# congkaishen/MotionPlanning

Measured on AMD Instinct MI355X. Metric: MPPI rollouts/s (K×H dyn+cost steps/s) at K=8192,H=50; 1/2/4/8 GPU, higher is better.
Workload: dtype f64

## Files before the change

motionplanning_amd/csrc/mppi.hip:

```cpp
#include "mppi_device.hpp"
#include "mppi_plan.hpp"
#include "runtime.hpp"

#include <hip/hip_ext.h>

#include <algorithm>
#include <cstdlib>
#include <type_traits>
#include <vector>

using namespace mpk;

namespace {

constexpr int NT = 256;
constexpr int RPB = NT / 2;

__device__ __forceinline__ double block_reduce_min(double v, double* sh) {
  for (int o = 32; o >= 1; o >>= 1) v = nanmin(v, __shfl_xor(v, o));
  const int w = threadIdx.x >> 6;
  __syncthreads();
  if ((threadIdx.x & 63) == 0) sh[w] = v;
  __syncthreads();
  double r = sh[0];
  for (int i = 1; i < (int)(blockDim.x >> 6); i++) r = nanmin(r, sh[i]);
  __syncthreads();
  return r;
}

__device__ __forceinline__ double block_reduce_sum(double v, double* sh) {
  for (int o = 32; o >= 1; o >>= 1) v = v + __shfl_xor(v, o);
  const int w = threadIdx.x >> 6;
  __syncthreads();
  if ((threadIdx.x & 63) == 0) sh[w] = v;
  __syncthreads();
  double r = sh[0];
  for (int i = 1; i < (int)(blockDim.x >> 6); i++) r = r + sh[i];
  __syncthreads();
  return r;
}

struct PlanArgs {
  const double* X0;
  const double* goal;
  const double* unom;
  const double* obs;
  const unsigned char* grid;
  const double* noise;
  double* ctrl_all;
  double* cost_all;
  unsigned char* feas_all;
  double* part;
  double* coll_traj;
  unsigned* tickets;
  int* flags;
  double* U_out;
  double* traj_out;
  double* cost_out;
  int* feas_out;
  int* rc_out;
  int* fc_out;
  int nb;
  int pstride;
  int lds_unom, lds_obs, lds_grid;
  int lds_cq;
  int lds_ctrl, lds_part;
  unsigned long long* stamps;
  int inline_noise;
  double* fin;
  int fin_stride;
  const int* live;
};

typedef unsigned mp_v4u __attribute__((ext_vector_type(4)));
typedef __attribute__((address_space(3))) mp_v4u mp_lds_v4u;
typedef __attribute__((address_space(3))) const unsigned long long mp_lds_cu64;

struct FinRec {
  int u, unom, x0, goal, obs, grid, ran, stride;
  __host__ __device__ FinRec(int H, int n_obs, int gbytes) {
    u = 0;
    unom = 2 * H;
    x0 = 4 * H;
    goal = x0 + 7;
    obs = goal + 2;
    grid = obs + 3 * n_obs;
    ran = grid + (gbytes + 7) / 8 + 1;
    stride = (ran + 2) & ~1;
  }
};
// ... 395 lines not shown
  for (int t = tid; t < H2; t += NT) {
    double acc = 0.0;
#pragma unroll 8
    for (int i = 0; i < nfull; i++) acc = acc + partS[(size_t)i * A.pstride + 4 + t] * scale[i];
    if (has_p) {
      double ap = 0.0;
      for (int r = 0; r < m - p0; r++) {
        const int kr = p0 + r, h = t >> 1;
        double u[2];
        double z[2];
        if (INL) {
          philox_normal2(P, (unsigned)s, (unsigned)kr, (unsigned)h, z);
        } else {
          const double2 zz = reinterpret_cast<const double2*>(noiseS)[(size_t)h * K + kr];
          z[0] = zz.x;
          z[1] = zz.y;
        }
        sample_ctrl(P, z, unom + 2 * h, u);
        ap = ap + sh_e[r] * u[t & 1];
      }
      acc = acc + ap * scale_p;
    }
    Ush[t] = acc * inv_eta;
  }
  __syncthreads();
  MP_STAMP(4);
  for (int t = tid; t < H2; t += NT) A.U_out[(size_t)s * H2 + t] = Ush[t];
  if (tid == 0) {
    A.rc_out[s] = m + 1;
    A.fc_out[s] = sh_fc;
    A.tickets[s] = 0u;
    if (rho != rho) atomicOr(A.flags, 1);
  }
  if (A.fin) {
    const FinRec R(H, P.n_obs, P.gnx * P.gny);
    double* rec = A.fin + (size_t)s * A.fin_stride;
    for (int t = tid; t < H2; t += NT) {
      rec[R.u + t] = Ush[t];
      rec[R.unom + t] = unom[t];
    }
    if (tid < 7) rec[R.x0 + tid] = X0[tid];
    if (tid == 0) rec[R.ran] = 1.0;
    if (tid < 2) rec[R.goal + tid] = goal[tid];
    for (int i = tid; i < 3 * P.n_obs; i += NT) rec[R.obs + i] = obs[i];
    if (grid) {
      const int gb = P.gnx * P.gny;
      const bool wide = LEAN || A.lds_grid >= 0;
      const int g7 = wide ? (int)(reinterpret_cast<size_t>(grid) & 7) : 0;
      unsigned char* rg = reinterpret_cast<unsigned char*>(rec + R.grid) + g7;
      if (tid == 0) rec[R.ran] = 1.0 + g7;
      if (wide) {
        const int head = min(gb, (8 - g7) & 7), n8 = (gb - head) >> 3;
        mp_lds_cu64* s8 = (mp_lds_cu64*)reinterpret_cast<const unsigned long long*>(grid + head);
        unsigned long long* d8 = reinterpret_cast<unsigned long long*>(rg + head);
        for (int i = tid; i < n8; i += NT) d8[i] = s8[i];
        if (tid < gb - 8 * n8) {
          const int q = tid < head ? tid : 8 * n8 + tid;
          rg[q] = grid[q];
        }
      } else {
        for (int i = tid; i < gb; i += NT) rg[i] = grid[i];
      }
    }
    MP_STAMP(5);
    return;
  }
  if (tid >= 64) return;
  __builtin_amdgcn_s_setprio(3);
  {
    auto ctrl = [&](int j, double* u) { u[0] = Ush[2 * j]; u[1] = Ush[2 * j + 1]; };
    auto store = [&](int, const double*) {};
    const TrajOut traj{A.traj_out + (size_t)s * (H + 1) * 7, 7, 1};
    int f2;
    const double c2 = rollout_pair(P, X0, goal, obs, grid, unom, tid & 1, ctrl, store, traj, &f2, atab);
    if (tid == 0) {
      A.cost_out[s] = c2;
      A.feas_out[s] = f2;
      if (c2 != c2) atomicOr(A.flags, 1);
    }
  }
  MP_STAMP(5);
}

__global__ __launch_bounds__(64) void final_rollout_kernel(MppiDev P, const double* fin, int fin_stride,
                                                           int grid_lds, double* traj_out, double* cost_out,
                                                           int* feas_out, int* flags) {
  extern __shared__ double fsh[];
  __shared__ double atab[kTabDoubles];
  const int s = blockIdx.x, tid = threadIdx.x, side = tid & 1, H = P.H;
  const FinRec R(H, P.n_obs, P.gnx * P.gny);
  const double* rec = fin + (size_t)s * fin_stride;
  const double ran = rec[R.ran];
  if (ran == 0.0) return;
  const int nw = grid_lds ? R.stride : R.grid;
  for (int i = tid; i < nw; i += 64) fsh[i] = rec[i];
  rollout_tab_fill(atab, P, threadIdx.x, blockDim.x);
  __syncthreads();
  const double* U = fsh + R.u;
  auto ctrl = [&](int j, double* u) { u[0] = U[2 * j]; u[1] = U[2 * j + 1]; };
  auto store = [&](int, const double*) {};
  const unsigned char* grid =
      P.gnx > 0 ? reinterpret_cast<const unsigned char*>((grid_lds ? fsh : rec) + R.grid) + ((int)ran - 1) : nullptr;
  const TrajOut traj{traj_out + (size_t)s * (H + 1) * 7, 7, 1};
  int f2;
  const double c2 = rollout_pair(P, fsh + R.x0, fsh + R.goal, P.n_obs > 0 ? fsh + R.obs : nullptr, grid,
                                 fsh + R.unom, side, ctrl, store, traj, &f2, atab);
  if (tid == 0) {
    cost_out[s] = c2;
    feas_out[s] = f2;
    if (c2 != c2) atomicOr(flags, 1);
  }
}

__global__ __launch_bounds__(NT) void rollout_kernel(MppiDev P, int K, const double* X0, const double* goal,
                                                     const double* ctrl, long long cs, const double* unom,
                                                     const double* obs, const unsigned char* grid, double* traj,
                                                     double* cost, unsigned char* feas, int nb) {
  const int H = P.H;
  const int s = blockIdx.x / nb, b = blockIdx.x % nb;
  const int tid = threadIdx.x, pair = tid >> 1, side = tid & 1;
  __shared__ double atab[kTabDoubles];
  rollout_tab_fill(atab, P, threadIdx.x, blockDim.x);
  __syncthreads();
  const int k = b * RPB + pair;
  const bool active = k < K;
  const int kk = active ? k : K - 1;
  const double* cu = ctrl + ((size_t)s * K + kk) * (cs ? (size_t)cs * H : 2);
  auto cf = [&](int j, double* u) {
    const double* q = cu + (size_t)j * cs;
    u[0] = q[0];
    u[1] = q[1];
  };
  auto store = [&](int, const double*) {};
  const TrajOut tr{(traj && active) ? traj + ((size_t)s * K + k) * (H + 1) * 7 : nullptr, 7, 1};
  int f;
  const double c = rollout_pair(P, X0 + 7 * s, goal + 2 * s, obs ? obs + (size_t)3 * P.n_obs * s : nullptr,
                                grid ? grid + (size_t)P.gnx * P.gny * s : nullptr,
                                unom ? unom + (size_t)2 * H * s : nullptr, side, cf, store, tr, &f, atab);
  if (active && side == 0) {
    cost[(size_t)s * K + k] = c;
    feas[(size_t)s * K + k] = (unsigned char)f;
  }
}

__global__ __launch_bounds__(NT) void argmin_kernel(int K, const double* cost, int* out) {
  __shared__ double sv[NT];
  __shared__ int si[NT];
  const int s = blockIdx.x;
  double bv = 0.0;
  int bi = -1;
  for (int i = threadIdx.x; i < K; i += NT) {
    const double v = cost[(size_t)s * K + i];
    if (bi < 0 || mpj_isless(v, bv)) { bv = v; bi = i; }
  }
  sv[threadIdx.x] = bv;
  si[threadIdx.x] = bi;
  __syncthreads();
  if (threadIdx.x == 0) {
    double v = sv[0];
    int ix = si[0];
    for (int t = 1; t < NT; t++) {
      if (si[t] < 0) continue;
      if (ix < 0 || mpj_isless(sv[t], v) || (!mpj_isless(v, sv[t]) && si[t] < ix)) { v = sv[t]; ix = si[t]; }
    }
    out[s] = ix;
  }
}

__global__ __launch_bounds__(64) void euler_kernel(int n, double* states, const double* ctrl, double dt,
                                                   int nsteps, double* his) {
  const int tid = blockIdx.x * 64 + threadIdx.x;
  const int v = tid >> 1, side = tid & 1;
  const int vv = v < n ? v : n - 1;
  __shared__ double atab[4 * MPJ_ATAN_ROWS];
  mpj_atan_rows_fill(atab, threadIdx.x, blockDim.x);
  __syncthreads();
  double x[7], d[7];
  for (int i = 0; i < 7; i++) x[i] = states[7 * vv + i];
  const double sr = ctrl[2 * vv], ax = ctrl[2 * vv + 1];
  for (int t = 0; t < nsteps; t++) {
    dyn_pair(x, sr, ax, d, side, atab);
    for (int i = 0; i < 7; i++) x[i] = x[i] + d[i] * dt;
    if (his && v < n && side == 0)
      for (int i = 0; i < 7; i++) his[((size_t)v * nsteps + t) * 7 + i] = x[i];
  }
  if (v < n && side == 0)
    for (int i = 0; i < 7; i++) states[7 * v + i] = x[i];
}

// ... 128 lines not shown
  D->gx0 = p->grid_x0; D->gy0 = p->grid_y0; D->gdx = p->grid_dx; D->gdy = p->grid_dy;
  D->noise_mode = p->noise_mode;
  D->ctrl_cost = p->ctrl_cost;
  D->seed = p->seed;
  D->offset = p->offset;
  D->scene_base = p->scene_base;
  return MP_OK;
}

using PlanFn = void (*)(MppiDev, PlanArgs);
struct PlanInst { int BT, LPR; bool inl, lean; PlanFn fn; };
#define MP_PLAN_INST(bt, lpr) \
  {bt, lpr, true, false, mppi_plan_kernel<bt, lpr, true>}, {bt, lpr, false, false, mppi_plan_kernel<bt, lpr, false>}
static const PlanInst kPlanKernels[] = {{256, 1, true, true, mppi_plan_kernel<256, 1, true, true>},
                                        {512, 1, true, true, mppi_plan_kernel<512, 1, true, true>},
                                        MP_PLAN_INST(256, 1), MP_PLAN_INST(256, 2), MP_PLAN_INST(512, 1), MP_PLAN_INST(512, 2)};
#undef MP_PLAN_INST
static PlanFn plan_kernel_for(int BT, int LPR, bool inl, bool lean) {
  for (const PlanInst& k : kPlanKernels)
    if (k.BT == BT && k.LPR == LPR && k.inl == inl && k.lean == lean) return k.fn;
  return nullptr;
}

struct PlanIn {
  const double *X0, *goal, *U_nom, *obstacles;
  const uint8_t* grid;
  const double* noise;
};
struct PlanOut {
  double *U, *traj, *cost;
  int32_t *feasible, *rc, *fc;
};
struct PlanColl {
  double *traj, *ctrl, *cost;
  uint8_t* feas;
};

static MppiShape plan_shape_for(const MppiDev& D, int S, const PlanIn& in, const PlanColl& coll) {
  const char* lpr_s = getenv("MPGPU_LPR");
  const char* lean_s = getenv("MPGPU_PLAN_LEAN");
  return mppi_plan_shape({S, D.K, D.H, D.n_obs, D.gnx, D.gny, D.in_flight, D.noise_mode == MP_NOISE_PHILOX,
                          D.ctrl_cost != 0, in.grid != nullptr, coll.traj && coll.ctrl, lpr_s ? atoi(lpr_s) : 0,
                          !(lean_s && lean_s[0] == '0' && !lean_s[1])});
}

static int plan_buffers(mp_ctx* ctx, const MppiDev& D, int S, const MppiShape& P, const PlanIn& in,
                        const PlanColl& coll, PlanArgs& A) {
  const int K = D.K, H = D.H;
  A.noise = nullptr;
  if (!A.inline_noise) {
    double* zh = (double*)mp_ws(ctx, WS_NOISE, sizeof(double) * (size_t)S * K * H * 2);
    if (!zh) return MP_ERR_NOMEM;
    const long long n = (long long)S * K * H;
    hipLaunchKernelGGL(noise_prep_kernel, dim3((unsigned)((n + 255) / 256)), dim3(256), 0, ctx->stream, D, S, in.noise,
                       zh);
    MP_HIP(ctx, hipGetLastError());
    A.noise = zh;
  }
  A.cost_all = coll.cost ? coll.cost : (double*)mp_ws(ctx, WS_MPPI_COST, sizeof(double) * (size_t)S * K);
  A.feas_all = coll.feas ? coll.feas : (unsigned char*)mp_ws(ctx, WS_MPPI_FEAS, (size_t)S * K);
  A.part = (double*)mp_ws(ctx, WS_MPPI_PART, sizeof(double) * (size_t)S * P.nb * P.pstride);
  if (!A.cost_all || !A.feas_all || !A.part) return MP_ERR_NOMEM;
  int st = mp_ticket_reserve(ctx, S);
  if (st) return st;
  A.tickets = ctx->tickets;
  A.flags = ctx->flags;
  A.ctrl_all = coll.ctrl;
  if (P.lds_ctrl < 0 && !A.ctrl_all) {
    A.ctrl_all = (double*)mp_ws(ctx, WS_IO14, sizeof(double) * (size_t)S * K * 2 * H);
    if (!A.ctrl_all) return MP_ERR_NOMEM;
  }
  return MP_OK;
}

static int plan_kernel_attrs(mp_ctx* ctx) {
  if (ctx->mppi_lds_attr) return MP_OK;
  MP_HIP(ctx, hipSetDevice(ctx->device));
  for (const PlanInst& k : kPlanKernels)
    MP_HIP(ctx, hipFuncSetAttribute((const void*)k.fn, hipFuncAttributeMaxDynamicSharedMemorySize, (int)kMaxLds));
  ctx->mppi_lds_attr = true;
  return MP_OK;
}

static int fin_slot_acquire(mp_ctx* ctx, const MppiDev& D, int S, PlanArgs& A, int* par) {
  int st = mp_side_init(ctx);
  if (st) return st;
  *par = ctx->fin_par;
  ctx->fin_par = (*par + 1) % MP_FIN_RING;
  const FinRec R(D.H, D.n_obs, D.gnx * D.gny);
  A.fin_stride = R.stride;
  for (int q = 0; q < MP_FIN_RING; q++)
    if (!mp_ws(ctx, WS_FIN0 + q, sizeof(double) * (size_t)S * R.stride)) return MP_ERR_NOMEM;
  A.fin = (double*)mp_ws(ctx, WS_FIN0 + *par, sizeof(double) * (size_t)S * R.stride);
  MP_HIP(ctx, hipEventSynchronize(ctx->ev_fin[*par]));
  return MP_OK;
}

static int plan_enqueue(mp_ctx* ctx, const MppiDev& D, int S, const MppiShape& P, const PlanArgs& A,
                        hipEvent_t* plan_done) {
  hipEvent_t t_start;
  mp_time_pair(ctx, &t_start, plan_done);
  void* args[] = {(void*)&D, (void*)&A};
  MP_HIP(ctx, hipExtLaunchKernel((const void*)plan_kernel_for(P.BT, P.LPR, A.inline_noise != 0, P.lean), dim3(S * P.nb),
                                 dim3(P.BT), args, sizeof(double) * P.lds_words, ctx->stream, t_start, *plan_done, 0));
  MP_HIP(ctx, hipGetLastError());
  return MP_OK;
}

static int final_rollout_enqueue(mp_ctx* ctx, const MppiDev& D, int S, const PlanArgs& A, int par,
                                 hipEvent_t plan_done, const PlanOut& out) {
  const FinRec R(D.H, D.n_obs, D.gnx * D.gny);
  const int grid_lds = (size_t)R.stride * 8 <= 64 * 1024;
  const size_t fsh = sizeof(double) * (size_t)(grid_lds ? R.stride : R.grid);
  MP_CHECK(ctx, fsh <= kMaxLds, "final rollout snapshot too large for LDS (%zu B)", fsh);
  if (!ctx->fin_lds_attr) {
    MP_HIP(ctx, hipSetDevice(ctx->device));
    MP_HIP(ctx, hipFuncSetAttribute((const void*)final_rollout_kernel, hipFuncAttributeMaxDynamicSharedMemorySize,
                                    (int)kMaxLds));
    ctx->fin_lds_attr = true;
  }
  if (!plan_done) {
    plan_done = ctx->ev_plan[par];
    MP_HIP(ctx, hipEventRecord(plan_done, ctx->stream));
  }
  MP_HIP(ctx, hipStreamWaitEvent(ctx->side, plan_done, 0));
  hipLaunchKernelGGL(final_rollout_kernel, dim3(S), dim3(64), fsh, ctx->side, D, A.fin, A.fin_stride, grid_lds,
                     out.traj, out.cost, out.feasible, ctx->flags);
  MP_HIP(ctx, hipGetLastError());
  MP_HIP(ctx, hipEventRecord(ctx->ev_fin[par], ctx->side));
  return MP_OK;
}

static bool stamps_on() {
  static const bool on = getenv("MPGPU_STAMPS") != nullptr;
  return on;
}

static int stamps_begin(mp_ctx* ctx, int nblk, PlanArgs& A) {
  const size_t bytes = sizeof(unsigned long long) * 32 * nblk;
  A.stamps = (unsigned long long*)mp_ws(ctx, WS_HA2, bytes);
  if (!A.stamps) return MP_ERR_NOMEM;
  MP_HIP(ctx, hipMemsetAsync(A.stamps, 0, bytes, ctx->stream));
  return MP_OK;
}

static void stamps_percentiles(const char* what, std::vector<double>& v) {
  std::sort(v.begin(), v.end());
  const size_t n = v.size();
  fprintf(stderr, " | %s p0/50/90/100 %.1f %.1f %.1f %.1f", what, v[0], v[n / 2], v[n * 9 / 10], v[n - 1]);
}

static int stamps_report(mp_ctx* ctx, const unsigned long long* stamps, int nblk) {
  std::vector<unsigned long long> h((size_t)32 * nblk);
  MP_HIP(ctx, hipMemcpyAsync(h.data(), stamps, h.size() * 8, hipMemcpyDeviceToHost, ctx->stream));
  MP_HIP(ctx, hipStreamSynchronize(ctx->stream));
  unsigned long long t0 = ~0ull, end = 0;
  double d01 = 0, d12 = 0, d23 = 0;
  int last = -1;
  for (int b = 0; b < nblk; b++) {
    const unsigned long long* q = &h[32 * b];
    t0 = q[0] < t0 ? q[0] : t0;
    d01 += (q[1] - q[0]) / 100.0; d12 += (q[2] - q[1]) / 100.0; d23 += (q[3] - q[2]) / 100.0;
    if (q[5]) last = b;
    end = q[5] > end ? q[5] : end;
    end = q[3] > end ? q[3] : end;
  }
  auto us = [&](unsigned long long t) { return (t - t0) / 100.0; };
  fprintf(stderr, "[stamps us] blocks=%d mean rollout %.2f partial %.2f ticket %.2f", nblk, d01 / nblk, d12 / nblk,
          d23 / nblk);
  std::vector<double> st, en, we;
  int hist[9] = {0};
  double sum[16] = {0}, mx[16] = {0};
  int cnt[16] = {0}, nbk[16] = {0};
  for (int b = 0; b < nblk; b++) {
    const unsigned long long* q = &h[32 * b];
    st.push_back(us(q[0]));
    en.push_back(us(q[1]));
    const int x = (int)(q[30] & 15);
    nbk[x]++;
    int on_simd[4] = {0, 0, 0, 0}, most = 0;
    for (int w = 0; w < 8; w++) {
      if (!q[8 + w]) continue;
      const double v = us(q[8 + w]);
      we.push_back(v);
      most = std::max(most, ++on_simd[(q[20 + w] >> 4) & 3]);
      sum[x] += v; cnt[x]++; mx[x] = std::max(mx[x], v);
    }
    hist[most]++;
  }
  stamps_percentiles("start", st);
  stamps_percentiles("p1-end", en);
  stamps_percentiles("wave-end", we);
  fprintf(stderr, " | blocks by max waves/SIMD 1:%d 2:%d 3:%d 4:%d", hist[1], hist[2], hist[3], hist[4]);
  fprintf(stderr, " | xcc(blocks mean/max):");
  for (int x = 0; x < 16; x++)
    if (cnt[x]) fprintf(stderr, " %d(%d %.1f/%.1f)", x, nbk[x], sum[x] / cnt[x], mx[x]);
  if (last >= 0) {
    const unsigned long long* q = &h[32 * last];
    fprintf(stderr, " | last block: start+%.2f combine %.2f final-rollout %.2f | total %.2f", us(q[0]),
            (q[4] - q[3]) / 100.0, (q[5] - q[4]) / 100.0, us(end));
  }
  fprintf(stderr, "\n");
  return MP_OK;
}

static int plan_launch(mp_ctx* ctx, const MppiDev& D, int S, const PlanIn& in, const PlanOut& out,
                       const PlanColl& coll, int final_stream, const int* live = nullptr) {
  const MppiShape P = plan_shape_for(D, S, in, coll);
  const size_t shmem = sizeof(double) * P.lds_words;
  MP_CHECK(ctx, shmem <= kMaxLds, "K/H/obstacles too large for one scene (dynamic LDS %zu B)", shmem);
  PlanArgs A;
  A.live = live;
  A.X0 = in.X0; A.goal = in.goal; A.unom = in.U_nom; A.obs = D.n_obs > 0 ? in.obstacles : nullptr;
  A.grid = D.gnx > 0 ? in.grid : nullptr;
  A.inline_noise = D.noise_mode == MP_NOISE_PHILOX;
  A.coll_traj = coll.traj;
  A.U_out = out.U; A.traj_out = out.traj; A.cost_out = out.cost; A.feas_out = out.feasible;
  A.rc_out = out.rc; A.fc_out = out.fc;
  A.nb = P.nb;
  A.pstride = P.pstride;
  A.lds_unom = P.lds_unom; A.lds_cq = P.lds_cq; A.lds_obs = P.lds_obs; A.lds_grid = P.lds_grid;
  A.lds_ctrl = P.lds_ctrl; A.lds_part = P.lds_part;
  int st = plan_buffers(ctx, D, S, P, in, coll, A);
  if (st || (st = plan_kernel_attrs(ctx))) return st;
  A.fin = nullptr;
  A.fin_stride = 0;
  int par = 0;
  if (final_stream && (st = fin_slot_acquire(ctx, D, S, A, &par))) return st;
  A.stamps = nullptr;
  if (stamps_on() && (st = stamps_begin(ctx, S * P.nb, A))) return st;
  hipEvent_t plan_done;
  if ((st = plan_enqueue(ctx, D, S, P, A, &plan_done))) return st;
  if (final_stream && (st = final_rollout_enqueue(ctx, D, S, A, par, plan_done, out))) return st;
  return stamps_on() ? stamps_report(ctx, A.stamps, S * P.nb) : MP_OK;
}

static int check_plan_inputs(mp_ctx* ctx, const mp_mppi_params* p, const PlanIn& in, bool outputs) {
  MP_CHECK(ctx, in.X0 && in.goal && in.U_nom && outputs, "required pointer is NULL");
  MP_CHECK(ctx, p->noise_mode != MP_NOISE_EXTERNAL || in.noise, "noise is NULL in MP_NOISE_EXTERNAL mode");
  MP_CHECK(ctx, p->n_obs == 0 || in.obstacles, "obstacles NULL with n_obs > 0");
  MP_CHECK(ctx, p->grid_nx == 0 || in.grid, "grid NULL with grid_nx > 0");
  return MP_OK;
}
static int check_plan_call(mp_ctx* ctx, const mp_mppi_params* p, int S, const PlanIn& in, const PlanOut& out) {
  MP_CHECK(ctx, S >= 1, "S (%d) must be >= 1", S);
  int st = check_plan_inputs(ctx, p, in, out.U && out.traj && out.cost && out.feasible && out.rc && out.fc);
  if (st) return st;
  MP_CHECK(ctx, p->final_stream == 0 || p->final_stream == 1, "final_stream (%d) must be 0 or 1", p->final_stream);
  return MP_OK;
}

static PlanIn upload_scene_inputs(mp_ctx* ctx, const mp_mppi_params* p, size_t n, const PlanIn& host, size_t noise_n,
                                  int* st) {
  PlanIn d;
  d.X0 = mp_upload(ctx, WS_IO0, host.X0, 7 * n, st);
  d.goal = mp_upload(ctx, WS_IO1, host.goal, 2 * n, st);
  d.U_nom = mp_upload(ctx, WS_IO2, host.U_nom, 2 * (size_t)p->H * n, st);
  d.obstacles = mp_upload(ctx, WS_IO3, p->n_obs ? host.obstacles : nullptr, 3 * (size_t)p->n_obs * n, st);
  d.grid = mp_upload(ctx, WS_IO4, p->grid_nx ? host.grid : nullptr, (size_t)p->grid_nx * p->grid_ny * n, st);
  d.noise = mp_upload(ctx, WS_IO5, p->noise_mode == MP_NOISE_EXTERNAL ? host.noise : nullptr, noise_n, st);
  return d;
}

}

extern "C" {

int mp_mppi_plan_dev(mp_ctx* ctx, const mp_mppi_params* p, int32_t S, const double* X0, const double* goal,
                     const double* U_nom, const double* obstacles, const uint8_t* grid, const double* noise,
                     double* U_out, double* traj_out, double* cost_out, int32_t* feasible_out,
                     int32_t* rollout_count_out, int32_t* feasible_count_out, double* coll_traj,
                     double* coll_ctrl, double* coll_cost, uint8_t* coll_feas) {
  if (!ctx) return MP_ERR_INVALID;
  MppiDev D;
  int st = make_dev_params(ctx, p, p ? p->K : 0, &D);
  if (st) return st;
  const PlanIn in = {X0, goal, U_nom, obstacles, grid, noise};
  const PlanOut out = {U_out, traj_out, cost_out, feasible_out, rollout_count_out, feasible_count_out};
  if ((st = check_plan_call(ctx, p, S, in, out))) return st;
  return plan_launch(ctx, D, S, in, out, {coll_traj, coll_ctrl, coll_cost, coll_feas}, p->final_stream);
}

int mp_mppi_plan(mp_ctx* ctx, const mp_mppi_params* p, int32_t S, const double* X0, const double* goal,
                 const double* U_nom, const double* obstacles, const uint8_t* grid, const double* noise,
                 double* U_out, double* traj_out, double* cost_out, int32_t* feasible_out,
// ... 340 lines not shown
```

motionplanning_amd/csrc/mppi_device.hpp:

```cpp
#pragma once
#include <hip/hip_runtime.h>

#include "../../include/mp_jlmath.h"

namespace mpk {

struct MppiDev {
  int K, H, FC, n_obs;
  double dt, lambda, nil;
  double L[4];
  double Si[4];
  double XL[7], XU[7], CL[2], CU[2];
  double slack, obs_pen;
  int gnx, gny;
  double gx0, gy0, gdx, gdy;
  int noise_mode, ctrl_cost;
  unsigned long long seed, offset;
  int scene_base;
  int in_flight;
};

__device__ __forceinline__ double pair_swap(double v) {
  const int lo = __builtin_amdgcn_mov_dpp(__double2loint(v), 0xB1, 0xF, 0xF, false);
  const int hi = __builtin_amdgcn_mov_dpp(__double2hiint(v), 0xB1, 0xF, 0xF, false);
  return __hiloint2double(hi, lo);
}

#ifndef MPPI_LIBM_OCML
#define MPPI_LIBM_OCML 0
#endif
#if MPPI_LIBM_OCML
#define TY_ATAN(x, tab) ::atan(x)
#define TY_SIN(x) ::sin(x)
#define TY_SINCOS(a, s, c) ::sincos((a), (s), (c))
#else
#define TY_ATAN(x, tab) mpj_atan_rows((x), (tab))
#define TY_SIN(x) mpj_sin_34(x)
#define TY_SINCOS(a, s, c) mpj_sincos_bl((a), (s), (c))
#endif
struct PairK {
  double kfz, tsg, lr, cown, cother, div, rdiv;
};
__device__ __forceinline__ PairK pair_k(int side) {
  const double la = 1.56, lb = 1.64, M = 2020.0, Izz = 4095.0;
  const double KFZF = 1018.28 / 2, KFZR = 963.34 / 2;
  PairK k;
  k.kfz = side ? KFZR : KFZF;
  k.tsg = side ? 1.0 : -1.0;
  k.lr = side ? -lb : la;
  k.cown = side ? -lb : 1.0;
  k.cother = side ? la : 1.0;
  k.div = side ? Izz : M;
  k.rdiv = mpj_rcp_nr(k.div);
  return k;
}
__device__ __forceinline__ void dyn_pair_sc(const double* x, double sr, double ax, double* d, int side,
                                            const double* atab, double sp, double cp, const PairK& pk) {
  const double g = 9.81, mu = 0.8, KFZX = 186.22;
  const double B = -10.4 / mu, C = 1.3, E = 0.1556;
  const double v = x[2], r = x[3], ux = x[5], sa = x[6];
  const double t = (ax - r * v) * KFZX;
  const double FZ = 2 * (pk.kfz * g + t * pk.tsg);
  const double alpha = TY_ATAN(mpj_div_g(v + pk.lr * r, ux + 0.01), atab) - (side ? 0.0 : sa);
  const double X1 = B * alpha;
  const double FY = mu * FZ * 1.0 * TY_SIN(C * TY_ATAN(X1 - E * (X1 - TY_ATAN(X1, atab)), atab));
  const double FYo = pair_swap(FY);
  const double uxc = MPJ_SEL(ux <= 0, 0.0, ux);
  d[0] = uxc * cp - v * sp;
  d[1] = uxc * sp + v * cp;
  const double q = mpj_div_gn(FY * pk.cown + FYo * pk.cother, pk.div, pk.rdiv, 1);
  const double qo = pair_swap(q);
  d[2] = (side ? qo : q) - r * uxc;
  d[3] = side ? q : qo;
  d[4] = r;
  d[5] = ax;
  d[6] = sr;
}
__device__ __forceinline__ void dyn_pair(const double* x, double sr, double ax, double* d, int side, const double* atab) {
  double sp, cp;
  TY_SINCOS(x[4], &sp, &cp);
  dyn_pair_sc(x, sr, ax, d, side, atab, sp, cp, pair_k(side));
}

struct LaneK {
  double rM, rI;
};
__device__ __forceinline__ LaneK lane_k() {
  LaneK k;
  k.rM = mpj_rcp_nr(2020.0);
  k.rI = mpj_rcp_nr(4095.0);
  return k;
}
__device__ __forceinline__ void dyn_lane(const double* x, double sr, double ax, double* d, const double* atab,
                                         const LaneK& lk) {
  const double la = 1.56, lb = 1.64, M = 2020.0, Izz = 4095.0, g = 9.81, mu = 0.8;
  const double KFZF = 1018.28 / 2, KFZR = 963.34 / 2, KFZX = 186.22;
  const double B = -10.4 / mu, C = 1.3, E = 0.1556;
  const double v = x[2], r = x[3], psi = x[4], ux = x[5], sa = x[6];
  const double t = (ax - r * v) * KFZX;
  const double FZf = 2 * (KFZF * g + -t), FZr = 2 * (KFZR * g + t);
  double qf, qr;
  mpj_div2_g(v + la * r, v + (-lb) * r, ux + 0.01, &qf, &qr);
  const double af = TY_ATAN(qf, atab) - sa;
  const double ar = TY_ATAN(qr, atab) - 0.0;
  const double Xf = B * af, Xr = B * ar;
  const double FY1 = mu * FZf * 1.0 * TY_SIN(C * TY_ATAN(Xf - E * (Xf - TY_ATAN(Xf, atab)), atab));
  const double FY2 = mu * FZr * 1.0 * TY_SIN(C * TY_ATAN(Xr - E * (Xr - TY_ATAN(Xr, atab)), atab));
  const double uxc = MPJ_SEL(ux <= 0, 0.0, ux);
  double sp, cp;
  TY_SINCOS(psi, &sp, &cp);
  d[0] = uxc * cp - v * sp;
  d[1] = uxc * sp + v * cp;
  d[2] = mpj_div_gn(FY1 + FY2, M, lk.rM, 1) - r * uxc;
  d[3] = mpj_div_gn(FY1 * la - FY2 * lb, Izz, lk.rI, 1);
  d[4] = r;
  d[5] = ax;
  d[6] = sr;
}

__device__ __forceinline__ double run_cost(const double* x, double sr, double ax) {
  const double y = x[1], v = x[2], r = x[3], sa = x[6];
  return v * v * 1 + 1 * (r * r) + 5 * (ax * ax) + 3 * (sr * sr) + 2 * (sa * sa) + 10 * (y * y);
}

struct GridK {
  double rx, ry;
  int ok;
};
template <int LPR = 2>
__device__ __forceinline__ GridK grid_k(const MppiDev& P, int side) {
  GridK g;
  g.rx = mpj_rcp_nr(LPR == 2 && side ? P.gdy : P.gdx);
  g.ry = mpj_rcp_nr(P.gdy);
  g.ok = P.gnx > 0 && !mpj_div_out(P.gdx) && !mpj_div_out(P.gdy);
  return g;
}
template <int LPR = 2, bool LEAN = false>
__device__ __forceinline__ double obstacle_cost(const MppiDev& P, const double* x, const double* obs,
                                                const unsigned char* grid, int* ok, int side, const GridK& gk) {
  double c = 0.0;
  for (int o = 0; !LEAN && o < P.n_obs; o++) {
    const double dx = x[0] - obs[3 * o], dy = x[1] - obs[3 * o + 1], R = obs[3 * o + 2];
    const int hit = dx * dx + dy * dy <= R * R;
    *ok &= !hit;
    c = (hit ? c + P.obs_pen : c);
  }
  if (LEAN || P.gnx > 0) {
    double fx, fy;
    if (LPR == 2) {
      const double f = mpj_div_gn(side ? x[1] - P.gy0 : x[0] - P.gx0, side ? P.gdy : P.gdx, gk.rx, gk.ok);
      const double fo = pair_swap(f);
      fx = side ? fo : f;
// ... 189 lines not shown
__device__ __forceinline__ void ctrl_cost_row(const MppiDev& P, double un0, double un1, double* t) {
  const double a0 = P.lambda * un0, a1 = P.lambda * un1;
  t[0] = __builtin_fma(P.Si[0], a0, P.Si[2] * a1);
  t[1] = __builtin_fma(P.Si[1], a0, P.Si[3] * a1);
}

template <int LPR = 2, bool LEAN = false, class CtrlFn, class StoreFn, class TrajT>
__device__ __forceinline__ double rollout_pair(const MppiDev& P, const double* X0, const double* goal,
                                               const double* obs, const unsigned char* grid,
                                               const double* unom, int side, CtrlFn ctrl, StoreFn store,
                                               const TrajT& traj_, int* feas, const double* atab,
                                               const double* cq = nullptr) {
  TrajT traj = traj_;
  double x[7];
#pragma unroll
  for (int i = 0; i < 7; i++) x[i] = X0[i];
  const PairK pk = pair_k(side);
  const LaneK lk = lane_k();
  const GridK gk = grid_k<LPR>(P, side);
  if (traj_on(traj)) store_state<LPR>(traj, 0, x, side);
  double sum = 0.0;
  int ok_all = 1;
  for (int j = 0; j < P.H; j++) {
    double u[2];
    ctrl(j, u);
    store(j, u);
    int okc = 1, okb = 1;
    double cc = 0.0, cb = 0.0;
    if (j > 0) {
      cc = obstacle_cost<LPR, LEAN>(P, x, obs, grid, &okc, side, gk);
      cb = LEAN ? bound_cost_lds(P, atab + kTabBnd, x, &okb) : bound_cost(P, atab + kTabBnd, x, &okb);
    }
    const double pc = run_cost(x, u[0], u[1]);
    double k1[7], k2[7], x2[7];
    if (LPR == 2) {
      const double psi2 = x[4] + x[3] * P.dt;
      double sn, cs;
      TY_SINCOS(side ? psi2 : x[4], &sn, &cs);
      const double so = pair_swap(sn), co = pair_swap(cs);
      dyn_pair_sc(x, u[0], u[1], k1, side, atab, side ? so : sn, side ? co : cs, pk);
#pragma unroll
      for (int i = 0; i < 7; i++) x2[i] = x[i] + k1[i] * P.dt;
      dyn_pair_sc(x2, u[0], u[1], k2, side, atab, side ? sn : so, side ? cs : co, pk);
    } else {
      dyn_lane(x, u[0], u[1], k1, atab, lk);
#pragma unroll
      for (int i = 0; i < 7; i++) x2[i] = x[i] + k1[i] * P.dt;
      dyn_lane(x2, u[0], u[1], k2, atab, lk);
    }
#pragma unroll
    for (int i = 0; i < 7; i++) x[i] = x[i] + P.dt * (k1[i] + k2[i]) / 2;
    double cj = pc + cb + cc;
    if (LEAN || P.ctrl_cost) {
      const double un0 = unom[2 * j], un1 = unom[2 * j + 1];
      double t[2];
      if (LEAN || cq) {
        t[0] = cq[2 * j];
        t[1] = cq[2 * j + 1];
      } else {
        ctrl_cost_row(P, un0, un1, t);
      }
      const double d0 = u[0] - un0, d1 = u[1] - un1;
      cj = cj + __builtin_fma(t[1], d1, t[0] * d0);
    }
    sum = sum + cj;
    ok_all &= okc & okb;
    if (traj_on(traj)) store_state<LPR>(traj, j + 1, x, side);
  }
  {
    int okc = 1, okb = 1;
    const double pc = run_cost(x, 0.0, 0.0);
    const double cc = obstacle_cost<LPR, LEAN>(P, x, obs, grid, &okc, side, gk);
    const double cb = LEAN ? bound_cost_lds(P, atab + kTabBnd, x, &okb) : bound_cost(P, atab + kTabBnd, x, &okb);
    sum = sum + (pc + cb + cc);
    ok_all &= okc & okb;
  }
  const double tx = x[0] - goal[0], ty = x[1] - goal[1];
  const double term = tx * tx + ty * ty;
  const double dx0 = X0[0] - goal[0], dy0 = X0[1] - goal[1];
  *feas = ok_all;
  return sum + term / (dx0 * dx0 + dy0 * dy0) * 10000.0;
}

__device__ __forceinline__ double nanmin(double a, double b) { return (a != a || a < b) ? a : b; }

}
```

motionplanning_amd/csrc/mppi_plan.hpp:

```cpp
#pragma once
#include <cstddef>

constexpr size_t kMaxLds = 146 * 1024;
constexpr size_t kCoLds = 70 * 1024;
constexpr int kGridPad = 32;

struct MppiShapeIn {
  int S, K, H, n_obs, gnx, gny;
  int in_flight;
  bool device_noise;
  bool ctrl_cost;
  bool grid;
  bool collect;
  int force_lpr;
  bool allow_lean;
};

struct MppiShape {
  int LPR, BT, RPB;
  int nb, pstride;
  bool lean;
  int lds_unom, lds_cq, lds_obs, lds_grid, lds_ctrl, lds_part;
  size_t lds_words;
};

inline MppiShape mppi_plan_shape(const MppiShapeIn& in) {
  const int S = in.S, K = in.K, H = in.H;
  MppiShape P;
  P.LPR = in.force_lpr == 1 || in.force_lpr == 2 ? in.force_lpr : ((size_t)S * K * in.in_flight >= 131072 ? 1 : 2);
  P.BT = P.LPR == 1 ? ((size_t)S * ((K + 511) / 512) >= 256 ? 512 : 256)
                    : ((size_t)S * ((K + 255) / 256) >= 256 ? 512 : 256);
  P.RPB = P.BT / P.LPR;
  P.nb = (K + P.RPB - 1) / P.RPB;
  P.pstride = 4 + 2 * H;
  size_t off = 2 * (size_t)H + P.nb;
  P.lds_unom = (int)off;
  off += 2 * (size_t)H;
  P.lds_cq = (int)off;
  off += 2 * (size_t)H;
  P.lds_obs = (int)off;
  off += 3 * (size_t)in.n_obs;
  const size_t gbytes = (size_t)in.gnx * in.gny;
  P.lds_grid = -1;
  if (in.gnx > 0 && off * 8 + gbytes + kGridPad <= 48 * 1024) {
    P.lds_grid = (int)off;
    off += (gbytes + kGridPad + 7) / 8;
  }
  const size_t ctrl_words = (size_t)P.RPB * (2 * (size_t)H + 1), part_words = (size_t)P.nb * P.pstride;
  P.lds_ctrl = P.lds_part = -1;
  const bool many = (size_t)S * P.nb > 256;
  const size_t budget = many ? kCoLds : kMaxLds;
  P.lean = in.allow_lean && P.LPR == 1 && (P.BT == 256 || P.BT == 512) && in.device_noise && in.n_obs == 0 &&
           in.grid && P.lds_grid >= 0 && in.ctrl_cost && in.collect && K < (1 << 27);
  const size_t both_words = ctrl_words > part_words ? ctrl_words : part_words;
  if (P.lean) {
    if ((off + part_words) * 8 <= budget) {
      P.lds_part = (int)off;
      off += part_words;
    }
  } else if ((off + both_words) * 8 <= budget) {
    P.lds_ctrl = P.lds_part = (int)off;
    off += both_words;
  } else if ((off + part_words) * 8 <= budget) {
    P.lds_part = (int)off;
    off += part_words;
  }
  P.lds_words = off;
  return P;
}
```

Measured before the change: 18.88 billion.

## Split final rollout into serial dynamics chain and parallel per-step position/cost rows

The final-rollout kernel gains a split path that is on by default when LDS allows. One lane pair integrates only the heading and velocity states and records them per step into an LDS table. All 64 lanes then compute the per-step position increments, a prefix sum rebuilds positions, and costs are evaluated in parallel across horizon steps. This shortens the serial chain in the tail kernel, at the cost of extra LDS use and syncs. It also adds env-gated timing counters around the final-slot event wait.

```diff
diff --git a/motionplanning_amd/csrc/mppi.hip b/motionplanning_amd/csrc/mppi.hip
--- a/motionplanning_amd/csrc/mppi.hip
+++ b/motionplanning_amd/csrc/mppi.hip
@@ -5,7 +5,10 @@
 #include <hip/hip_ext.h>
 
 #include <algorithm>
+#include <atomic>
+#include <chrono>
 #include <cstdlib>
+#include <cstring>
 #include <type_traits>
 #include <vector>
 
@@ -567,6 +570,7 @@
   MP_STAMP(5);
 }
 
+template <bool SPLIT>
 __global__ __launch_bounds__(64) void final_rollout_kernel(MppiDev P, const double* fin, int fin_stride,
                                                            int grid_lds, double* traj_out, double* cost_out,
                                                            int* feas_out, int* flags) {
@@ -587,9 +591,17 @@
   const unsigned char* grid =
       P.gnx > 0 ? reinterpret_cast<const unsigned char*>((grid_lds ? fsh : rec) + R.grid) + ((int)ran - 1) : nullptr;
   const TrajOut traj{traj_out + (size_t)s * (H + 1) * 7, 7, 1};
+  const double* obs = P.n_obs > 0 ? fsh + R.obs : nullptr;
   int f2;
-  const double c2 = rollout_pair(P, fsh + R.x0, fsh + R.goal, P.n_obs > 0 ? fsh + R.obs : nullptr, grid,
-                                 fsh + R.unom, side, ctrl, store, traj, &f2, atab);
+  double c2;
+  if constexpr (SPLIT) {
+    double* tab = fsh + nw;
+    rollout_chain(P, fsh + R.x0, side, tid, ctrl, atab, tab);
+    __syncthreads();
+    c2 = rollout_rows(P, fsh + R.x0, fsh + R.goal, obs, grid, fsh + R.unom, tid, ctrl, traj.p, &f2, atab, tab);
+  } else {
+    c2 = rollout_pair(P, fsh + R.x0, fsh + R.goal, obs, grid, fsh + R.unom, side, ctrl, store, traj, &f2, atab);
+  }
   if (tid == 0) {
     cost_out[s] = c2;
     feas_out[s] = f2;
@@ -884,6 +896,26 @@
   return MP_OK;
 }
 
+static bool stamps_fin_only() {
+  static const bool on = [] {
+    const char* s = getenv("MPGPU_STAMPS");
+    return s && !strcmp(s, "fin");
+  }();
+  return on;
+}
+static bool stamps_on() {
+  static const bool on = getenv("MPGPU_STAMPS") != nullptr && !stamps_fin_only();
+  return on;
+}
+struct FinWaits {
+  std::atomic<long long> calls{0}, waited{0}, ns{0};
+};
+static FinWaits g_fin_waits;
+static void fin_waits_print() {
+  fprintf(stderr, "[stamps fin] fin_slot_acquire: %lld calls, %lld waited, %.3f ms in all\n", g_fin_waits.calls.load(),
+          g_fin_waits.waited.load(), g_fin_waits.ns.load() * 1e-6);
+}
+
 static int fin_slot_acquire(mp_ctx* ctx, const MppiDev& D, int S, PlanArgs& A, int* par) {
   int st = mp_side_init(ctx);
   if (st) return st;
@@ -894,7 +926,20 @@
   for (int q = 0; q < MP_FIN_RING; q++)
     if (!mp_ws(ctx, WS_FIN0 + q, sizeof(double) * (size_t)S * R.stride)) return MP_ERR_NOMEM;
   A.fin = (double*)mp_ws(ctx, WS_FIN0 + *par, sizeof(double) * (size_t)S * R.stride);
+  if (!stamps_on() && !stamps_fin_only()) {
+    MP_HIP(ctx, hipEventSynchronize(ctx->ev_fin[*par]));
+    return MP_OK;
+  }
+  static const int at_exit = stamps_fin_only() ? atexit(fin_waits_print) : 0;
+  (void)at_exit;
+  const bool busy = hipEventQuery(ctx->ev_fin[*par]) == hipErrorNotReady;
+  const auto t0 = std::chrono::steady_clock::now();
   MP_HIP(ctx, hipEventSynchronize(ctx->ev_fin[*par]));
+  g_fin_waits.calls++;
+  if (busy) {
+    g_fin_waits.waited++;
+    g_fin_waits.ns += std::chrono::duration_cast<std::chrono::nanoseconds>(std::chrono::steady_clock::now() - t0).count();
+  }
   return MP_OK;
 }
 
@@ -912,13 +957,19 @@
 static int final_rollout_enqueue(mp_ctx* ctx, const MppiDev& D, int S, const PlanArgs& A, int par,
                                  hipEvent_t plan_done, const PlanOut& out) {
   const FinRec R(D.H, D.n_obs, D.gnx * D.gny);
-  const int grid_lds = (size_t)R.stride * 8 <= 64 * 1024;
-  const size_t fsh = sizeof(double) * (size_t)(grid_lds ? R.stride : R.grid);
-  MP_CHECK(ctx, fsh <= kMaxLds, "final rollout snapshot too large for LDS (%zu B)", fsh);
+  const char* split_s = getenv("MPGPU_FINAL_SPLIT");
+  const char* lds_s = getenv("MPGPU_FINAL_LDS");
+  const MppiFinalShape F = mppi_final_shape(D.H, (size_t)R.stride, (size_t)R.grid,
+                                            !(split_s && split_s[0] == '0' && !split_s[1]),
+                                            lds_s ? (size_t)strtoull(lds_s, nullptr, 10) : kMaxLds);
+  const int grid_lds = F.grid_lds;
+  MP_CHECK(ctx, F.snap_words * 8 <= kMaxLds, "final rollout snapshot too large for LDS (%zu B)", F.snap_words * 8);
+  const size_t fsh = sizeof(double) * F.lds_words;
+  const auto kernel = F.split ? final_rollout_kernel<true> : final_rollout_kernel<false>;
   if (!ctx->fin_lds_attr) {
     MP_HIP(ctx, hipSetDevice(ctx->device));
-    MP_HIP(ctx, hipFuncSetAttribute((const void*)final_rollout_kernel, hipFuncAttributeMaxDynamicSharedMemorySize,
-                                    (int)kMaxLds));
+    for (const auto k : {final_rollout_kernel<true>, final_rollout_kernel<false>})
+      MP_HIP(ctx, hipFuncSetAttribute((const void*)k, hipFuncAttributeMaxDynamicSharedMemorySize, (int)kMaxLds));
     ctx->fin_lds_attr = true;
   }
   if (!plan_done) {
@@ -926,16 +977,11 @@
     MP_HIP(ctx, hipEventRecord(plan_done, ctx->stream));
   }
   MP_HIP(ctx, hipStreamWaitEvent(ctx->side, plan_done, 0));
-  hipLaunchKernelGGL(final_rollout_kernel, dim3(S), dim3(64), fsh, ctx->side, D, A.fin, A.fin_stride, grid_lds,
-                     out.traj, out.cost, out.feasible, ctx->flags);
+  hipLaunchKernelGGL(kernel, dim3(S), dim3(64), fsh, ctx->side, D, A.fin, A.fin_stride, grid_lds, out.traj, out.cost,
+                     out.feasible, ctx->flags);
   MP_HIP(ctx, hipGetLastError());
   MP_HIP(ctx, hipEventRecord(ctx->ev_fin[par], ctx->side));
   return MP_OK;
-}
-
-static bool stamps_on() {
-  static const bool on = getenv("MPGPU_STAMPS") != nullptr;
-  return on;
 }
 
 static int stamps_begin(mp_ctx* ctx, int nblk, PlanArgs& A) {
@@ -1003,6 +1049,7 @@
             (q[4] - q[3]) / 100.0, (q[5] - q[4]) / 100.0, us(end));
   }
   fprintf(stderr, "\n");
+  fin_waits_print();
   return MP_OK;
 }
 
diff --git a/motionplanning_amd/csrc/mppi_device.hpp b/motionplanning_amd/csrc/mppi_device.hpp
--- a/motionplanning_amd/csrc/mppi_device.hpp
+++ b/motionplanning_amd/csrc/mppi_device.hpp
@@ -2,6 +2,7 @@
 #include <hip/hip_runtime.h>
 
 #include "../../include/mp_jlmath.h"
+#include "mppi_plan.hpp"
 
 namespace mpk {
 
@@ -54,6 +55,7 @@
   k.rdiv = mpj_rcp_nr(k.div);
   return k;
 }
+template <bool CHAIN = false>
 __device__ __forceinline__ void dyn_pair_sc(const double* x, double sr, double ax, double* d, int side,
                                             const double* atab, double sp, double cp, const PairK& pk) {
   const double g = 9.81, mu = 0.8, KFZX = 186.22;
@@ -66,8 +68,10 @@
   const double FY = mu * FZ * 1.0 * TY_SIN(C * TY_ATAN(X1 - E * (X1 - TY_ATAN(X1, atab)), atab));
   const double FYo = pair_swap(FY);
   const double uxc = MPJ_SEL(ux <= 0, 0.0, ux);
-  d[0] = uxc * cp - v * sp;
-  d[1] = uxc * sp + v * cp;
+  if (!CHAIN) {
+    d[0] = uxc * cp - v * sp;
+    d[1] = uxc * sp + v * cp;
+  }
   const double q = mpj_div_gn(FY * pk.cown + FYo * pk.cother, pk.div, pk.rdiv, 1);
   const double qo = pair_swap(q);
   d[2] = (side ? qo : q) - r * uxc;
@@ -423,6 +427,122 @@
   return sum + term / (dx0 * dx0 + dy0 * dy0) * 10000.0;
 }
 
+constexpr int kFinAux = 7;
+
+template <class CtrlFn>
+__device__ __forceinline__ void rollout_chain(const MppiDev& P, const double* X0, int side, int lane, CtrlFn ctrl,
+                                              const double* atab, double* tab) {
+  const PairK pk = pair_k(side);
+  double x[7] = {0.0, 0.0, X0[2], X0[3], X0[4], X0[5], X0[6]};
+  for (int j = 0; j < P.H; j++) {
+    double u[2];
+    ctrl(j, u);
+    double k1[7], k2[7], x2[7] = {0.0, 0.0};
+    dyn_pair_sc<true>(x, u[0], u[1], k1, side, atab, 0.0, 0.0, pk);
+#pragma unroll
+    for (int i = 2; i < 7; i++) x2[i] = x[i] + k1[i] * P.dt;
+    dyn_pair_sc<true>(x2, u[0], u[1], k2, side, atab, 0.0, 0.0, pk);
+    if (lane == 0) {
+      double* row = tab + (size_t)kFinCols * j;
+#pragma unroll
+      for (int i = 2; i < 7; i++) row[i] = x[i];
+      row[kFinAux] = k1[2];
+    }
+#pragma unroll
+    for (int i = 2; i < 7; i++) x[i] = x[i] + P.dt * (k1[i] + k2[i]) / 2;
+  }
+  if (lane == 0) {
+#pragma unroll
+    for (int i = 2; i < 7; i++) tab[(size_t)kFinCols * P.H + i] = x[i];
+  }
+}
+
+template <class CtrlFn>
+__device__ __forceinline__ double rollout_rows(const MppiDev& P, const double* X0, const double* goal,
+                                               const double* obs, const unsigned char* grid, const double* unom,
+                                               int lane, CtrlFn ctrl, double* rows, int* feas, const double* atab,
+                                               double* tab) {
+  const int H = P.H;
+  for (int j0 = 0; j0 < H; j0 += 64) {
+    const int j = j0 + lane, jj = j < H ? j : H - 1;
+    const double* row = tab + (size_t)kFinCols * jj;
+    double u[2];
+    ctrl(jj, u);
+    const double v = row[2], r = row[3], psi = row[4], ux = row[5];
+    const double v2 = v + row[kFinAux] * P.dt, psi2 = psi + r * P.dt, ux2 = ux + u[1] * P.dt;
+    double s1, c1, s2, c2;
+    TY_SINCOS(psi, &s1, &c1);
+    TY_SINCOS(psi2, &s2, &c2);
+    const double uxc = MPJ_SEL(ux <= 0, 0.0, ux), uxc2 = MPJ_SEL(ux2 <= 0, 0.0, ux2);
+    const double k10 = uxc * c1 - v * s1, k11 = uxc * s1 + v * c1;
+    const double k20 = uxc2 * c2 - v2 * s2, k21 = uxc2 * s2 + v2 * c2;
+    if (j < H) {
+      double* nx = tab + (size_t)kFinCols * (j + 1);
+      nx[0] = P.dt * (k10 + k20) / 2;
+      nx[1] = P.dt * (k11 + k21) / 2;
+    }
+  }
+  __syncthreads();
+  if (lane == 0) {
+    double px = X0[0], py = X0[1];
+    tab[0] = px;
+    tab[1] = py;
+    for (int j = 1; j <= H; j++) {
+      double* row = tab + (size_t)kFinCols * j;
+      px = px + row[0];
+      py = py + row[1];
+      row[0] = px;
+      row[1] = py;
+    }
+  }
+  __syncthreads();
+  const GridK gk = grid_k<1>(P, 0);
+  int ok = 1;
+  for (int j0 = 0; j0 <= H; j0 += 64) {
+    const int j = j0 + lane, jj = j < H ? j : H, jc = jj < H ? jj : H - 1;
+    const bool step = jj < H;
+    double* row = tab + (size_t)kFinCols * jj;
+    double x[7], u[2];
+#pragma unroll
+    for (int i = 0; i < 7; i++) x[i] = row[i];
+    ctrl(jc, u);
+    u[0] = step ? u[0] : 0.0;
+    u[1] = step ? u[1] : 0.0;
+    int okc = 1, okb = 1;
+    double cc = obstacle_cost<1>(P, x, obs, grid, &okc, 0, gk);
+    double cb = bound_cost_lds(P, atab + kTabBnd, x, &okb);
+    if (jj == 0) {
+      cc = 0.0;
+      cb = 0.0;
+      okc = okb = 1;
+    }
+    const double pc = run_cost(x, u[0], u[1]);
+    double cj = pc + cb + cc;
+    if (P.ctrl_cost) {
+      const double un0 = unom[2 * jc], un1 = unom[2 * jc + 1];
+      double t[2];
+      ctrl_cost_row(P, un0, un1, t);
+      const double d0 = u[0] - un0, d1 = u[1] - un1;
+      const double cu = cj + __builtin_fma(t[1], d1, t[0] * d0);
+      cj = step ? cu : cj;
+    }
+    if (j <= H) {
+      row[kFinAux] = cj;
+      ok &= okc & okb;
+#pragma unroll
+      for (int i = 0; i < 7; i++) st_state(rows + (size_t)7 * j + i, x[i]);
+    }
+  }
+  __syncthreads();
+  double sum = 0.0;
+  for (int j = 0; j <= H; j++) sum = sum + tab[(size_t)kFinCols * j + kFinAux];
+  const double tx = tab[(size_t)kFinCols * H] - goal[0], ty = tab[(size_t)kFinCols * H + 1] - goal[1];
+  const double term = tx * tx + ty * ty;
+  const double dx0 = X0[0] - goal[0], dy0 = X0[1] - goal[1];
+  *feas = __all(ok) ? 1 : 0;
+  return sum + term / (dx0 * dx0 + dy0 * dy0) * 10000.0;
+}
+
 __device__ __forceinline__ double nanmin(double a, double b) { return (a != a || a < b) ? a : b; }
 
 }
diff --git a/motionplanning_amd/csrc/mppi_plan.hpp b/motionplanning_amd/csrc/mppi_plan.hpp
--- a/motionplanning_amd/csrc/mppi_plan.hpp
+++ b/motionplanning_amd/csrc/mppi_plan.hpp
@@ -68,3 +68,26 @@
   P.lds_words = off;
   return P;
 }
+
+constexpr int kFinCols = 8;
+constexpr size_t kFinGridLds = 64 * 1024;
+
+struct MppiFinalShape {
+  bool grid_lds;
+  bool split;
+  size_t snap_words;
+  size_t chain_words;
+  size_t lds_words;
+};
+
+inline MppiFinalShape mppi_final_shape(int H, size_t rec_words, size_t rec_grid_at, bool allow_split,
+                                       size_t budget = kMaxLds) {
+  MppiFinalShape F;
+  F.grid_lds = rec_words * 8 <= kFinGridLds;
+  F.snap_words = F.grid_lds ? rec_words : rec_grid_at;
+  const size_t chain = ((size_t)H + 1) * kFinCols;
+  F.split = allow_split && (F.snap_words + chain) * 8 <= (budget < kMaxLds ? budget : kMaxLds);
+  F.chain_words = F.split ? chain : 0;
+  F.lds_words = F.snap_words + F.chain_words;
+  return F;
+}
```

New measurement: 18.43 billion. 2.4% lower.
